# NVlabs/FoundationPose

Measured on AMD Instinct MI355X. Metric: pose-hypotheses/sec (raster+refine+score), 252 hyp x 160x160 @ 640x480 RGB-D, higher is better.
Workload: dtype f16

## Files before the change

### foundationpose_amd/csrc/conv_sw.hip

```cpp
#include <hip/hip_fp16.h>
#include <stdlib.h>
#include <string.h>
#include <type_traits>
#include "igemm_common.h"
#include "igemm_epilogue.h"

#ifdef FP_PROFILE_BUILD
__device__ unsigned long long sw_dbg[8];
extern "C" int fp_dbg_conv_sw(unsigned long long* out, int reset) {
  if (reset) { unsigned long long z[8] = {0, 0, 0, 0, 0, 0, ~0ull, 0}; return (int)hipMemcpyToSymbol(HIP_SYMBOL(sw_dbg), z, sizeof(z)); }
  return (int)hipMemcpyFromSymbol(out, HIP_SYMBOL(sw_dbg), 8 * sizeof(unsigned long long));
}
extern "C" int fp_dbg_conv_sw_epilogue(unsigned long long* out, int reset) {
  if (reset) { unsigned long long z[8] = {0, 0, 0, 0, 0, 0, 0, 0}; return (int)hipMemcpyToSymbol(HIP_SYMBOL(ig_epi_dbg), z, sizeof(z)); }
  return (int)hipMemcpyFromSymbol(out, HIP_SYMBOL(ig_epi_dbg), 8 * sizeof(unsigned long long));
}
#define SW_CLK(t) const unsigned long long t = wall_clock64()
#else
#define SW_CLK(t)
#endif

#ifndef SW_DEFAULT_VARIANT
#define SW_DEFAULT_VARIANT 0
#endif

namespace {

constexpr int SW_BK = 32, SW_NSTW = 4;
constexpr int sw_prows(int BM) { return BM == 256 ? 512 : 768; }

template <int N>
__device__ __forceinline__ void sw_wait_vm() {
  static_assert(N >= 0 && N < 64, "vmcnt is a 6-bit field");
  asm volatile("s_waitcnt vmcnt(%0)" ::"n"(N) : "memory");
}

typedef float sw_float4 __attribute__((ext_vector_type(4)));
__device__ __forceinline__ void sw_mfma16(sw_float4& acc, const half8& a, const half8& b) {
  asm volatile("v_mfma_f32_16x16x32_f16 %0, %1, %2, %0" : "+v"(acc) : "v"(a), "v"(b));
}

__device__ __forceinline__ int sw_q(const IgemmGeom& g, int m) {
  const int b = ig_fastdiv(m, g.mulP, g.shrP);
  const int r = m - b * g.HoWo;
  const int oy = ig_fastdiv(r, g.mulW, g.shrW);
  const int ox = r - oy * g.Wo;
  return (b * g.Hp + oy) * g.Wp + ox;
}

template <int BM, int BN, int TM, bool S16>
__global__ __launch_bounds__(512, 1) void k_conv_sw(IgemmParams p) {
  constexpr int BK = SW_BK, NW = 8, THREADS = 512;
  constexpr int NWN = BN / 64;
  static_assert((BM / (32 * TM)) * NWN == NW, "8 waves");
  constexpr int ROWB = BK * 2;
  constexpr int W_BYTES = BN * ROWB;
  constexpr int SW_PROWS = sw_prows(BM);
  constexpr int SW_PATCH_BYTES = SW_PROWS * ROWB;
  constexpr int WI = BN / 16 / NW;
  constexpr int PI = SW_PROWS / 16 / NW;
  static_assert(WI >= 1 && PI >= 1 && PI <= 7 && SW_PROWS == PI * 16 * NW, "tile shape");
  constexpr int STAGES_BYTES = 2 * SW_PATCH_BYTES + SW_NSTW * W_BYTES;
  constexpr int LDS_MAIN = ig_lds_main_slim<BM, BN>(STAGES_BYTES);
  auto swz = [](int row) { return (row >> 2) & 3; };
  auto swzp = [](int row) { return S16 ? (row >> 1) & 2 : (row >> 2) & 3; };
  extern __shared__ __attribute__((aligned(16))) unsigned char smem[];
  SW_CLK(t_start);
  unsigned char* const patch = smem;
  unsigned char* const wring = smem + 2 * SW_PATCH_BYTES;
  const int tid = threadIdx.x, lane = tid & 63;
  const int wid = __builtin_amdgcn_readfirstlane(tid >> 6);
  const int grp = wid >> 2;
  const int wm = wid / NWN, wn = wid - wm * NWN;
  float* bias_lds = reinterpret_cast<float*>(smem + LDS_MAIN);

  const int tiles_n = p.N / BN;
  const int nwg = gridDim.x;
  const int xcd = blockIdx.x & 7, loc = blockIdx.x >> 3;
  const int qd8 = nwg >> 3, r8 = nwg & 7;
  const int tile = (xcd < r8 ? xcd * (qd8 + 1) : r8 * (qd8 + 1) + (xcd - r8) * qd8) + loc;
  const int bm = tile / tiles_n, bn = tile - bm * tiles_n;
  const int m0 = bm * BM, n0 = bn * BN;
  const int Cin = p.Cin, Ktot = 9 * Cin, Wp = p.in.Wp;
  const int ncc = Cin / BK;
  ig_bias_to_lds(p, n0, bias_lds, wid, lane);

  const int q0 = sw_q(p.in, m0);
  const int qmax = (p.M / p.in.HoWo) * p.in.Hp * Wp - 1;
  unsigned poff32[PI], woff32[WI];
#pragma unroll
  for (int j = 0; j < PI; ++j) {
    const int row = (wid * PI + j) * 16 + (lane >> 2);
    const int c = (lane & 3) ^ swzp(row);
    int q = q0 + row;
    q = q < qmax ? q : qmax;
    poff32[j] = (unsigned)(((long long)q * p.in.cstride + p.in.coff + c * 8) * 2);
  }
#pragma unroll
  for (int j = 0; j < WI; ++j) {
    const int row = (wid * WI + j) * 16 + (lane >> 2);
    const int c = (lane & 3) ^ swz(row);
    woff32[j] = (unsigned)((((size_t)(n0 + row) * Ktot) + c * 8) * 2);
  }
  const bool wpk = (BN == 128) && p.Wpk != nullptr;
  if (wpk) {
#pragma unroll
    for (int j = 0; j < WI; ++j) woff32[j] = (unsigned)(((wid * WI + j) * 64 + lane) * 16);
  }
  const int wpk_base = wpk ? bn * (ncc * 9) * W_BYTES : 0;
  const __amdgpu_buffer_rsrc_t rsA = __builtin_amdgcn_make_buffer_rsrc(const_cast<_Float16*>(p.A), 0, 0x7FFFFFFF, 0x00020000);
  const __amdgpu_buffer_rsrc_t rsW = __builtin_amdgcn_make_buffer_rsrc(const_cast<_Float16*>(wpk ? p.Wpk : p.Wt), 0, 0x7FFFFFFF, 0x00020000);

  auto stage_patch = [&](int cc, int j) {
    unsigned char* dst = patch + (cc & 1) * SW_PATCH_BYTES + (wid * PI + j) * 1024;
    __builtin_amdgcn_raw_ptr_buffer_load_lds(rsA, (__attribute__((address_space(3))) void*)dst, 16, (int)poff32[j],
                                             cc * (BK * 2), 0, 0);
  };
  auto stage_w = [&](int cc, int tap, int slot) {
    const int wsoff = wpk ? wpk_base + (cc * 9 + tap) * W_BYTES : (tap * Cin + cc * BK) * 2;
    unsigned char* dst = wring + slot * W_BYTES + wid * (WI * 1024);
#pragma unroll
    for (int j = 0; j < WI; ++j)
      __builtin_amdgcn_raw_ptr_buffer_load_lds(rsW, (__attribute__((address_space(3))) void*)(dst + j * 1024), 16,
                                               (int)woff32[j], wsoff, 0, 0);
  };

  constexpr int NFA = S16 ? 2 * TM : TM, NFW = S16 ? 4 : 2;
  constexpr int FR = S16 ? 16 : 32;
  typedef float float4_ __attribute__((ext_vector_type(4)));
  typedef typename std::conditional<S16, float4_, float16_>::type acc_t;
  acc_t acc[NFW][NFA];
#pragma unroll
  for (int i = 0; i < NFW; ++i)
#pragma unroll
    for (int j = 0; j < NFA; ++j)
#pragma unroll
      for (int e = 0; e < (S16 ? 4 : 16); ++e) acc[i][j][e] = 0.f;

  const int frow = lane & (FR - 1), fhalf = lane >> (S16 ? 4 : 5);
  int arow[NFA], w_off[2][2];
#pragma unroll
  for (int t = 0; t < NFA; ++t) {
    int m = m0 + wm * (32 * TM) + t * FR + frow;
    m = m < p.M ? m : p.M - 1;
    arow[t] = sw_q(p.in, m) - q0;
    if constexpr (S16) arow[t] = (arow[t] << 6) + (fhalf << 4);
  }
  if constexpr (S16) {
    const int quad = (0x1320 >> (4 * (frow >> 2))) & 3;
#pragma unroll
    for (int t = 0; t < 4; ++t) {
      const int rw = wn * 64 + t * 16 + 4 * quad + (frow & 3);
      w_off[t >> 1][t & 1] = rw * ROWB + ((fhalf ^ swz(rw)) << 4);
    }
  } else {
#pragma unroll
    for (int t = 0; t < 2; ++t) {
      const int rw = wn * 64 + t * 32 + frow;
#pragma unroll
      for (int kk = 0; kk < 2; ++kk) w_off[t][kk] = rw * ROWB + (((2 * kk + fhalf) ^ swz(rw)) << 4);
    }
  }

#pragma unroll
  for (int j = 0; j < PI; ++j) stage_patch(0, j);
  stage_w(0, 0, 0);
  stage_w(0, 1, 1);
  stage_w(0, 2, 2);
  sw_wait_vm<2 * WI>();
  __builtin_amdgcn_s_barrier();
  SW_CLK(t_cold);
  if (grp) __builtin_amdgcn_s_barrier();

  half8 fa[2][TM], fw[2][2];
  static_assert(TM == 4, "the fragment addresses of the next tap are computed behind the MFMA groups of a k-step, one per group of four");
  int anext[NFA], aflip[NFA];
#pragma unroll
  for (int t = 0; t < NFA; ++t) {
    anext[t] = S16 ? arow[t] : (arow[t] << 6) + ((fhalf ^ swz(arow[t])) << 4);
    aflip[t] = S16 ? (arow[t] >> 3) & 32 : 0;
  }
  auto kstep = [&](int cc, auto tap_c, auto last_c) {
    constexpr int T = decltype(tap_c)::value;
    constexpr bool LAST = decltype(last_c)::value;
    constexpr int ky = T / 3, kx = T - 3 * ky;
    const int s = cc * 9 + T;
    const unsigned char* pb = patch + (cc & 1) * SW_PATCH_BYTES;
    const unsigned char* wb = wring + (s & (SW_NSTW - 1)) * W_BYTES;
    const int shift = ky * Wp + kx;
    if constexpr (S16) {
#pragma unroll
      for (int t = 0; t < NFA; ++t) fa[t >> 2][t & 3] = *reinterpret_cast<const half8*>(pb + (anext[t] ^ aflip[t]));
#pragma unroll
      for (int t = 0; t < 4; ++t) fw[t >> 1][t & 1] = *reinterpret_cast<const half8*>(wb + w_off[t >> 1][t & 1]);
    } else {
#pragma unroll
      for (int t = 0; t < TM; ++t) {
        const int a0 = anext[t];
        fa[0][t] = *reinterpret_cast<const half8*>(pb + a0);
        fa[1][t] = *reinterpret_cast<const half8*>(pb + (a0 ^ 32));
      }
#pragma unroll
      for (int kk = 0; kk < 2; ++kk)
#pragma unroll
        for (int t = 0; t < 2; ++t) fw[kk][t] = *reinterpret_cast<const half8*>(wb + w_off[t][kk]);
    }
    (void)shift;
    if constexpr (!LAST) {
      if constexpr (T < PI) stage_patch(cc + 1, T);
      if constexpr (T + 3 < 9) stage_w(cc, T + 3, (s + 3) & (SW_NSTW - 1));
      else stage_w(cc + 1, T - 6, (s + 3) & (SW_NSTW - 1));
      constexpr int NP = (T < PI ? 1 : 0) + ((T >= 1 && T - 1 < PI) ? 1 : 0);
      sw_wait_vm<2 * WI + NP>();
    } else {
      if constexpr (T + 3 < 9) stage_w(cc, T + 3, (s + 3) & (SW_NSTW - 1));
      constexpr int NYOUNGER = T <= 5 ? 2 : (T == 6 ? 1 : 0);
      sw_wait_vm<NYOUNGER * WI>();
    }
    asm volatile("s_waitcnt lgkmcnt(0)" ::: "memory");
    __builtin_amdgcn_sched_barrier(0);
    __builtin_amdgcn_s_barrier();
    __builtin_amdgcn_sched_barrier(0);
    __builtin_amdgcn_s_setprio(1);
    {
      constexpr int TN = (T + 1) % 9, kyn = TN / 3, kxn = TN - 3 * kyn;
      const int shift_n = kyn * Wp + kxn;
      if constexpr (S16) {
        int sh = shift_n << 6;
        asm volatile("" : "+s"(sh));
#pragma unroll
        for (int i = 0; i < 4; ++i)
#pragma unroll
          for (int jh = 0; jh < 2; ++jh) {
            const int t = i * 2 + jh;
            int x, y;
            sw_mfma16(acc[i][jh * 4 + 0], fw[i >> 1][i & 1], fa[jh][0]);
            asm volatile("v_add_u32 %0, %1, %2" : "=v"(x) : "s"(sh), "v"(arow[t]));
            sw_mfma16(acc[i][jh * 4 + 1], fw[i >> 1][i & 1], fa[jh][1]);
            asm volatile("v_lshrrev_b32 %0, 3, %1" : "=v"(y) : "v"(x));
            sw_mfma16(acc[i][jh * 4 + 2], fw[i >> 1][i & 1], fa[jh][2]);
            asm volatile("v_and_b32 %0, 32, %0" : "+v"(y));
            sw_mfma16(acc[i][jh * 4 + 3], fw[i >> 1][i & 1], fa[jh][3]);
            anext[t] = x; aflip[t] = y;
          }
      } else {
#pragma unroll
      for (int kk = 0; kk < 2; ++kk)
#pragma unroll
        for (int i = 0; i < 2; ++i) {
#pragma unroll
          for (int j = 0; j < TM; ++j)
            acc[i][j] = __builtin_amdgcn_mfma_f32_32x32x16_f16(fw[kk][i], fa[kk][j], acc[i][j], 0, 0, 0);
          const int t = kk * 2 + i;
          {
            int ar = arow[t];
            asm volatile("" : "+v"(ar));
            const int pr = ar + shift_n;
            anext[t] = (pr << 6) + ((fhalf ^ swz(pr)) << 4);
          }
        }
      }
    }
    __builtin_amdgcn_s_setprio(0);
    __builtin_amdgcn_sched_barrier(0);
    __builtin_amdgcn_s_barrier();
    __builtin_amdgcn_sched_barrier(0);
  };
  auto chunk = [&](int cc, auto last_c) {
    kstep(cc, std::integral_constant<int, 0>{}, last_c);
    kstep(cc, std::integral_constant<int, 1>{}, last_c);
    kstep(cc, std::integral_constant<int, 2>{}, last_c);
    kstep(cc, std::integral_constant<int, 3>{}, last_c);
    kstep(cc, std::integral_constant<int, 4>{}, last_c);
    kstep(cc, std::integral_constant<int, 5>{}, last_c);
    kstep(cc, std::integral_constant<int, 6>{}, last_c);
    kstep(cc, std::integral_constant<int, 7>{}, last_c);
    kstep(cc, std::integral_constant<int, 8>{}, last_c);
  };
  for (int cc = 0; cc + 1 < ncc; ++cc) chunk(cc, std::false_type{});
  chunk(ncc - 1, std::true_type{});
  if (!grp) __builtin_amdgcn_s_barrier();
  __syncthreads();
  SW_CLK(t_loop);
  ig_epilogue<BM, BN, TM, THREADS, 0, true>(p, acc, smem, m0, n0, wm, wn, tid, lane, bias_lds);
#ifdef FP_PROFILE_BUILD
  asm volatile("s_waitcnt vmcnt(0)" ::: "memory");
  SW_CLK(t_end);
  if (tid == 0) {
    atomicAdd(&sw_dbg[0], t_cold - t_start); atomicAdd(&sw_dbg[1], t_loop - t_cold); atomicAdd(&sw_dbg[2], t_end - t_loop);
    atomicAdd(&sw_dbg[3], 1ull); atomicMin(&sw_dbg[6], t_start); atomicMax(&sw_dbg[7], t_end);
  }
#endif
}

constexpr int LS_PROWS = 448, LS_NSTW = 3;

template <int BM, int BN, int TM>
__global__ __launch_bounds__(256, 2) void k_conv_sw_ls(IgemmParams p) {
  constexpr int BK = SW_BK, NW = 4, THREADS = 256;
  constexpr int NWN = BN / 64;
  static_assert((BM / (32 * TM)) * NWN == NW, "4 waves");
  constexpr int ROWB = BK * 2;
  constexpr int W_BYTES = BN * ROWB;
  constexpr int PATCH_BYTES = LS_PROWS * ROWB;
  constexpr int WI = BN / 16 / NW;
  constexpr int PI = LS_PROWS / 16 / NW;
  static_assert(WI >= 1 && PI >= 1 && PI <= 8 && LS_PROWS == PI * 16 * NW, "tile shape");
  constexpr int STAGES_BYTES = 2 * PATCH_BYTES + LS_NSTW * W_BYTES;
  static_assert(STAGES_BYTES >= BM * BN * 2 + BM * 16 + IG_BIAS_LDS, "the epilogue tile, its tables and the vectors reuse the staging area");
  auto swz = [](int row) { return (row >> 2) & 3; };
  extern __shared__ __attribute__((aligned(16))) unsigned char smem[];
  unsigned char* const patch = smem;
  unsigned char* const wring = smem + 2 * PATCH_BYTES;
  const int tid = threadIdx.x, lane = tid & 63;
  const int wid = __builtin_amdgcn_readfirstlane(tid >> 6);
  const int wm = wid / NWN, wn = wid - wm * NWN;

  const int tiles_n = p.N / BN;
  const int nwg = gridDim.x;
  const int xcd = blockIdx.x & 7, loc = blockIdx.x >> 3;
  const int qd8 = nwg >> 3, r8 = nwg & 7;
  const int tile = (xcd < r8 ? xcd * (qd8 + 1) : r8 * (qd8 + 1) + (xcd - r8) * qd8) + loc;
  const int bm = tile / tiles_n, bn = tile - bm * tiles_n;
  const int m0 = bm * BM, n0 = bn * BN;
  const int Cin = p.Cin, Ktot = 9 * Cin, Wp = p.in.Wp;
  const int ncc = Cin / BK;

  const int q0 = sw_q(p.in, m0);
  const int qmax = (p.M / p.in.HoWo) * p.in.Hp * Wp - 1;
  unsigned poff32[PI], woff32[WI];
#pragma unroll
  for (int j = 0; j < PI; ++j) {
    const int row = (wid * PI + j) * 16 + (lane >> 2);
    const int c = (lane & 3) ^ swz(row);
    int q = q0 + row;
    q = q < qmax ? q : qmax;
    poff32[j] = (unsigned)(((long long)q * p.in.cstride + p.in.coff + c * 8) * 2);
  }
#pragma unroll
  for (int j = 0; j < WI; ++j) {
    const int row = (wid * WI + j) * 16 + (lane >> 2);
    const int c = (lane & 3) ^ swz(row);
    woff32[j] = (unsigned)((((size_t)(n0 + row) * Ktot) + c * 8) * 2);
  }
  const __amdgpu_buffer_rsrc_t rsA = __builtin_amdgcn_make_buffer_rsrc(const_cast<_Float16*>(p.A), 0, 0x7FFFFFFF, 0x00020000);
  const __amdgpu_buffer_rsrc_t rsW = __builtin_amdgcn_make_buffer_rsrc(const_cast<_Float16*>(p.Wt), 0, 0x7FFFFFFF, 0x00020000);

  auto stage_patch = [&](int cc, int j) {
    unsigned char* dst = patch + (cc & 1) * PATCH_BYTES + (wid * PI + j) * 1024;
    __builtin_amdgcn_raw_ptr_buffer_load_lds(rsA, (__attribute__((address_space(3))) void*)dst, 16, (int)poff32[j],
                                             cc * (BK * 2), 0, 0);
  };
  auto stage_w = [&](int cc, int tap, int slot) {
    const int wsoff = (tap * Cin + cc * BK) * 2;
    unsigned char* dst = wring + slot * W_BYTES + wid * (WI * 1024);
#pragma unroll
    for (int j = 0; j < WI; ++j)
      __builtin_amdgcn_raw_ptr_buffer_load_lds(rsW, (__attribute__((address_space(3))) void*)(dst + j * 1024), 16,
                                               (int)woff32[j], wsoff, 0, 0);
  };

  float16_ acc[2][TM];
#pragma unroll
  for (int i = 0; i < 2; ++i)
#pragma unroll
    for (int j = 0; j < TM; ++j)
#pragma unroll
      for (int e = 0; e < 16; ++e) acc[i][j][e] = 0.f;

  const int frow = lane & 31, fhalf = lane >> 5;
  int arow[TM], w_off[2][2];
#pragma unroll
  for (int t = 0; t < TM; ++t) {
// ... 67 lines not shown
    kstep(cc, std::integral_constant<int, 0>{}, last_c, first_c);
    kstep(cc, std::integral_constant<int, 1>{}, last_c, std::false_type{});
    kstep(cc, std::integral_constant<int, 2>{}, last_c, std::false_type{});
    kstep(cc, std::integral_constant<int, 3>{}, last_c, std::false_type{});
    kstep(cc, std::integral_constant<int, 4>{}, last_c, std::false_type{});
    kstep(cc, std::integral_constant<int, 5>{}, last_c, std::false_type{});
    kstep(cc, std::integral_constant<int, 6>{}, last_c, std::false_type{});
    kstep(cc, std::integral_constant<int, 7>{}, last_c, std::false_type{});
    kstep(cc, std::integral_constant<int, 8>{}, last_c, std::false_type{});
  };
  chunk(0, std::false_type{}, std::true_type{});
  for (int cc = 1; cc + 1 < ncc; ++cc) chunk(cc, std::false_type{}, std::false_type{});
  chunk(ncc - 1, std::true_type{}, std::false_type{});
  __syncthreads();
  float* bias_lds = reinterpret_cast<float*>(smem + BM * BN * 2 + BM * 16);
  ig_bias_to_lds(p, n0, bias_lds, wid, lane);
  asm volatile("s_waitcnt vmcnt(0)" ::: "memory");
  ig_epilogue<BM, BN, TM, THREADS, 0>(p, acc, smem, m0, n0, wm, wn, tid, lane, bias_lds);
}

template <int BM, int BN, int TM>
int sw_ls_launch(const IgemmParams& p, hipStream_t stream) {
  constexpr int LDS = 2 * LS_PROWS * SW_BK * 2 + LS_NSTW * BN * SW_BK * 2;
  static_assert(2 * LDS <= 160 * 1024, "two workgroups per CU");
  const long long tiles = (long long)fp_cdiv(p.M, BM) * (p.N / BN);
  FP_REQUIRE(tiles < (1ll << 31), "fp_igemm_f16_fwd: too many tiles");
  FP_SET_MAX_LDS((k_conv_sw_ls<BM, BN, TM>), LDS);
  hipLaunchKernelGGL((k_conv_sw_ls<BM, BN, TM>), dim3((unsigned)tiles), dim3(256), LDS, stream, p);
  FP_CHECK_LAUNCH("fp_igemm_f16_fwd(conv_sw_ls)");
  return FP_OK;
}

constexpr int sw_lds_bytes(int BM, int BN) {
  return (BM == 256 ? ig_lds_main_slim<256, 256>(2 * sw_prows(256) * SW_BK * 2 + SW_NSTW * 256 * SW_BK * 2)
                    : ig_lds_main_slim<512, 128>(2 * sw_prows(512) * SW_BK * 2 + SW_NSTW * 128 * SW_BK * 2)) + IG_BIAS_LDS;
}

template <int BM, int BN, int TM, bool S16>
int sw_launch(const IgemmParams& p, hipStream_t stream) {
  static_assert((BM == 256 && BN == 256) || (BM == 512 && BN == 128), "tile shapes of sw_lds_bytes");
  constexpr int LDS = sw_lds_bytes(BM, BN);
  static_assert(LDS <= 160 * 1024, "does not fit the 160 KiB LDS");
  const long long tiles = (long long)fp_cdiv(p.M, BM) * (p.N / BN);
  FP_REQUIRE(tiles < (1ll << 31), "fp_igemm_f16_fwd: too many tiles");
  FP_SET_MAX_LDS((k_conv_sw<BM, BN, TM, S16>), LDS);
  hipLaunchKernelGGL((k_conv_sw<BM, BN, TM, S16>), dim3((unsigned)tiles), dim3(512), LDS, stream, p);
  FP_CHECK_LAUNCH("fp_igemm_f16_fwd(conv_sw)");
  return FP_OK;
}

}

static int sw_span(const IgemmGeom& g, int BM) {
  const int row_cross = (BM - 1) / g.Wo + 1, img_cross = (BM - 1) / g.HoWo + 1;
  return (BM - 1) + 2 * row_cross + (2 * g.Wp + 2) * img_cross + 2 * g.Wp + 3;
}

static int sw_variant(const IgemmParams& p) {
  int v = SW_DEFAULT_VARIANT;
#ifdef FP_PROFILE_BUILD
  static int forced = -2;
  if (forced == -2) {
    const char* e = getenv("FP_CONV_SW");
    forced = e ? (!strcmp(e, "ls") ? 1 : (!strcmp(e, "pp") ? 0 : -1)) : -1;
  }
  if (forced >= 0) v = forced;
#endif
  if (v == 2) v = p.Cin <= 128 ? 1 : 0;
  if (v == 3) v = p.Cin <= 256 ? 1 : 0;
  if (v == 1 && sw_span(p.in, 256) > LS_PROWS) v = 0;
  return v;
}

#ifndef SW_FORCE_512
#define SW_FORCE_512 1
#endif
static bool sw_use_256(const IgemmParams& p) { return (p.N % 256) == 0 && (!SW_FORCE_512 || p.M < 2 * 512); }
static int sw_tile_rows(const IgemmParams& p) { return sw_variant(p) == 1 ? 256 : (sw_use_256(p) ? 256 : 512); }

bool fp_conv3x3_sw_applicable(const IgemmParams& p) {
  const IgemmGeom& g = p.in;
  if (p.taps != 9 || g.stride != 1 || g.off != 0 || g.bsplit != 0) return false;
  if (g.HoWo % g.Wo != 0 || g.Wp != g.Wo + 2 || g.Hp != g.HoWo / g.Wo + 2) return false;
  const int BM = sw_tile_rows(p);
  if (p.M % g.HoWo != 0 || p.M < 2 * BM) return false;
  if (p.Cin % 64 != 0 || p.N % 128 != 0) return false;
  const long long bytes = (long long)(p.M / g.HoWo) * g.Hp * g.Wp * g.cstride * 2;
  if (bytes >= (1ll << 31)) return false;
  const IgemmGeom& o = p.out;
  const long long imgs = o.bsplit > 0 ? o.bsplit : p.M / g.HoWo, groups = o.bsplit > 0 ? (p.M / g.HoWo) / o.bsplit + 1 : 0;
  if (imgs * o.Hp * o.Wp * o.cstride + o.coff + groups * (long long)o.cgroup >= (1ll << 31)) return false;
  if (p.R) {
    const IgemmGeom& r = p.res;
    const long long rimgs = r.bsplit > 0 ? r.bsplit : p.M / g.HoWo, rgroups = r.bsplit > 0 ? (p.M / g.HoWo) / r.bsplit + 1 : 0;
    if (rimgs * r.Hp * r.Wp * r.cstride + r.coff + rgroups * (long long)r.cgroup >= (1ll << 31)) return false;
  }
  return sw_span(g, BM) <= (sw_variant(p) == 1 ? LS_PROWS : sw_prows(BM));
}

int fp_conv3x3_sw_tile_rows(const IgemmParams& p) { return sw_tile_rows(p); }

extern "C" int fp_conv3x3_sw_lds_bytes(void) { return sw_lds_bytes(512, 128); }

int fp_conv3x3_sw_launch(const IgemmParams& p, hipStream_t stream) {
  if (sw_variant(p) == 1) return sw_ls_launch<256, 128, 4>(p, stream);
  if (sw_use_256(p)) return p.mfma16 ? sw_launch<256, 256, 4, true>(p, stream) : sw_launch<256, 256, 4, false>(p, stream);
  return p.mfma16 ? sw_launch<512, 128, 4, true>(p, stream) : sw_launch<512, 128, 4, false>(p, stream);
}

__global__ __launch_bounds__(256) void k_pack_conv3x3_tiles(const _Float16* __restrict__ w, _Float16* __restrict__ out, int N, int Cin) {
  const int nk = 9 * (Cin / 32);
  const long long total = (long long)N * nk * 4;
  const long long q = (long long)blockIdx.x * 256 + threadIdx.x;
  if (q >= total) return;
  const int pc = (int)(q & 3);
  const int r = (int)((q >> 2) & 127);
  const long long blk = q >> 9;
  const int s = (int)(blk % nk), bn = (int)(blk / nk);
  const int cc = s / 9, tap = s - 9 * cc;
  const int lc = pc ^ ((r >> 2) & 3);
  const half8 v = *reinterpret_cast<const half8*>(w + (size_t)(bn * 128 + r) * (9 * Cin) + tap * Cin + cc * 32 + lc * 8);
  *reinterpret_cast<half8*>(out + q * 8) = v;
}

extern "C" int fp_pack_conv3x3_tiles_f16(const void* w, void* w_tiles, int N, int Cin, void* stream) {
  FP_REQUIRE(w && w_tiles && w != w_tiles, "fp_pack_conv3x3_tiles_f16: NULL tensor or in-place repack");
  FP_REQUIRE(N > 0 && N % 128 == 0 && Cin > 0 && Cin % 32 == 0, "fp_pack_conv3x3_tiles_f16: N=%d must be a multiple of 128, Cin=%d of 32", N, Cin);
  FP_REQUIRE((((size_t)w | (size_t)w_tiles) & 15) == 0, "fp_pack_conv3x3_tiles_f16: tensors must be 16-byte aligned");
  const long long total = (long long)N * 9 * (Cin / 32) * 4;
  hipLaunchKernelGGL(k_pack_conv3x3_tiles, dim3((unsigned)((total + 255) / 256)), dim3(256), 0, (hipStream_t)stream, (const _Float16*)w,
                     (_Float16*)w_tiles, N, Cin);
  FP_CHECK_LAUNCH("fp_pack_conv3x3_tiles_f16");
  return FP_OK;
}
```

### foundationpose_amd/csrc/igemm_common.h

```cpp
#pragma once
#include <hip/hip_fp16.h>
#include "fp_common.h"

typedef _Float16 half8 __attribute__((ext_vector_type(8)));
typedef _Float16 half4 __attribute__((ext_vector_type(4)));
typedef float float16_ __attribute__((ext_vector_type(16)));

#define IG_BK 64
#ifndef SW_DEFAULT_MFMA16
#define SW_DEFAULT_MFMA16 1
#endif

struct IgemmGeom {
  int HoWo, Wo;
  int Hp, Wp;
  int stride;
  int off;
  int cstride;
  int coff;
  int bsplit;
  int cgroup;
  unsigned mulP, shrP;
  unsigned mulW, shrW;
  unsigned mulB, shrB;
};

static inline void ig_fastdiv_init(int d, unsigned* mul, unsigned* shr) {
  if (d <= 1) { *mul = 0; *shr = 0; return; }
  int lg = 0;
  while ((1u << lg) < (unsigned)d) ++lg;
  const int p = 31 + lg;
  *mul = (unsigned)(((1ull << p) + (unsigned)d - 1) / (unsigned)d);
  *shr = (unsigned)(p - 32);
}
__device__ __forceinline__ int ig_fastdiv(int n, unsigned mul, unsigned shr) {
  return mul ? (int)(__umulhi((unsigned)n, mul) >> shr) : n;
}

struct IgemmParams {
  const _Float16* A;
  const _Float16* Wt;
  const _Float16* Wpk;
  const float* bias;
  const float* bn_scale;
  const float* bn_shift;
  const _Float16* R;
  _Float16* Y;
  const float* pe;
  _Float16* Ype;
  int pe_period;
  int M, N, Cin, taps;
  int relu;
  int round_acc;
  IgemmGeom in, out, res;
  int mfma16;
  int epi;
  unsigned pe_mul, pe_shr;
  float* slab;
  int nsplit;
};

#define IG_EPI_SPEC 1
#define IG_EPI_ROUND_ACC 2
#define IG_EPI_BIAS 4
#define IG_EPI_BN 8
#define IG_EPI_RES 16
#define IG_EPI_RELU 32
#define IG_EPI_PE 64
#define IG_EPI_CONV (IG_EPI_SPEC | IG_EPI_ROUND_ACC | IG_EPI_BIAS | IG_EPI_RELU)

__device__ __forceinline__ long long ig_row_off(const IgemmGeom& g, int m) {
  const int b = ig_fastdiv(m, g.mulP, g.shrP);
  const int r = m - b * g.HoWo;
  const int oy = ig_fastdiv(r, g.mulW, g.shrW);
  const int ox = r - oy * g.Wo;
  int bb = b, cg = 0;
  if (g.bsplit > 0) { cg = ig_fastdiv(b, g.mulB, g.shrB); bb = b - cg * g.bsplit; }
  return (((long long)bb * g.Hp + (oy * g.stride + g.off)) * g.Wp + (ox * g.stride + g.off)) * g.cstride + g.coff +
         (long long)cg * g.cgroup;
}
```

### foundationpose_amd/csrc/igemm_epilogue.h

```cpp
#pragma once
#include <type_traits>
#include "igemm_common.h"

#ifdef FP_PROFILE_BUILD
static __device__ unsigned long long ig_epi_dbg[8];
#define IG_CLK(t) const unsigned long long t = wall_clock64()
#else
#define IG_CLK(t)
#endif

#define IG_VEC_FLOATS 256
#define IG_BIAS_LDS (3 * IG_VEC_FLOATS * 4)

template <int BM, int BN>
constexpr int ig_lds_main(int stage_bytes) {
  return stage_bytes > BM * BN * 2 + BM * 16 ? stage_bytes : BM * BN * 2 + BM * 16;
}

template <int BM, int BN>
constexpr int ig_lds_main_slim(int stage_bytes) {
  return stage_bytes > BM * BN * 2 + BM * 4 ? stage_bytes : BM * BN * 2 + BM * 4;
}
#define IG_ROW_NONE ((int)0x80000000)

typedef float ig_float4 __attribute__((ext_vector_type(4)));
struct IgEpiArgs {
  IgemmGeom out, res;
  const _Float16* R;
  _Float16* Y;
  const float* pe;
  _Float16* Ype;
  int pe_period;
  unsigned pe_mul, pe_shr;
  int N;
};

template <typename T>
__device__ __forceinline__ T* ig_uniform_ptr(const T* ptr) {
  const unsigned long long a = reinterpret_cast<unsigned long long>(ptr);
  const unsigned lo = __builtin_amdgcn_readfirstlane((unsigned)a), hi = __builtin_amdgcn_readfirstlane((unsigned)(a >> 32));
  return reinterpret_cast<T*>(((unsigned long long)hi << 32) | lo);
}

__device__ __forceinline__ half8 ig_relu8(const half8& v) {
  typedef _Float16 half2_ __attribute__((ext_vector_type(2)));
  half8 r;
#pragma unroll
  for (int e = 0; e < 4; ++e) {
    const half2_ x = {v[2 * e], v[2 * e + 1]};
    half2_ y;
    asm("v_pk_max_f16 %0, %1, 0" : "=v"(y) : "v"(x));
    r[2 * e] = y[0]; r[2 * e + 1] = y[1];
  }
  return r;
}

template <int BM, int BN, int TM, int THREADS, bool SLIM, int EPI, typename Acc>
__device__ __forceinline__ void ig_epilogue_spec(const IgEpiArgs& p, Acc& acc, unsigned char* smem, int m0, int n0,
                                                 int wm, int wn, int tid, int lane, const float* bias_lds) {
  constexpr bool S16 = std::is_same<Acc, ig_float4[4][2 * TM]>::value;
  static_assert(S16 || std::is_same<Acc, float16_[2][TM]>::value, "accumulator layout");
  static_assert((EPI & IG_EPI_SPEC) && (EPI & IG_EPI_BIAS), "a layer kind with a bias");
  constexpr bool ROUND_ACC = (EPI & IG_EPI_ROUND_ACC) != 0, HAS_BN = (EPI & IG_EPI_BN) != 0, RES = (EPI & IG_EPI_RES) != 0;
  constexpr bool RELU = (EPI & IG_EPI_RELU) != 0, PE = (EPI & IG_EPI_PE) != 0;
  static_assert(ROUND_ACC || !HAS_BN, "BatchNorm follows the conv rounding");
  constexpr int CPR = BN / 8;
  constexpr int NIT = (BM * CPR) / THREADS;
  constexpr int RPI = THREADS / CPR;
  static_assert(THREADS % CPR == 0 && RPI % 16 == 0 && NIT * RPI == BM, "the store loop's swizzle term must not depend on the iteration");
  constexpr int ROWB = 2 * BN;
  typedef float float4_ __attribute__((ext_vector_type(4)));
  typedef _Float16 half2_ __attribute__((ext_vector_type(2)));
  typedef unsigned uint4_ __attribute__((ext_vector_type(4)));
  unsigned char* E = smem;
  long long* rowY = reinterpret_cast<long long*>(smem + BM * ROWB);
  long long* rowR = SLIM ? reinterpret_cast<long long*>(smem) : rowY + BM;
  int* rowY32 = reinterpret_cast<int*>(smem + BM * ROWB);
  const long long baseY = SLIM ? ig_row_off(p.out, m0) + n0 : 0;
  IG_CLK(te0);
  for (int r = tid; r < BM; r += THREADS) {
    const int m = m0 + r;
    if constexpr (SLIM) rowY32[r] = (int)(ig_row_off(p.out, m) + n0 - baseY);
    else rowY[r] = ig_row_off(p.out, m) + n0;
    if constexpr (RES) rowR[r] = ig_row_off(p.res, m) + n0;
  }
  __syncthreads();
  IG_CLK(te1);
  const int ml0 = tid / CPR, ch = tid % CPR;
  half8 rv[RES ? NIT : 1];
  if constexpr (RES) {
    if constexpr (SLIM) {
      const __amdgpu_buffer_rsrc_t rsR = __builtin_amdgcn_make_buffer_rsrc(ig_uniform_ptr(p.R), 0, -1, 0x00020000);
      const int* rR = reinterpret_cast<const int*>(rowR + ml0);
#pragma unroll
      for (int it = 0; it < NIT; ++it)
        rv[it] = __builtin_bit_cast(half8, __builtin_amdgcn_raw_buffer_load_b128(rsR, (int)(((unsigned)rR[it * RPI * 2] + ch * 8) << 1), 0, 0));
      __builtin_amdgcn_sched_barrier(0);
      asm volatile("s_waitcnt lgkmcnt(0)" ::: "memory");
      __builtin_amdgcn_s_barrier();
      __builtin_amdgcn_sched_barrier(0);
    } else {
      const long long* rR = rowR + ml0;
#pragma unroll
      for (int it = 0; it < NIT; ++it) rv[it] = *reinterpret_cast<const half8*>(p.R + rR[it * RPI] + ch * 8);
    }
  }
  IG_CLK(te2);
  struct Vecs { float4_ bv, sc, sh; half2_ b01, b23; };
  auto vecs = [&](int nl) {
    Vecs c;
    c.bv = *reinterpret_cast<const float4_*>(bias_lds + nl);
    c.b01 = half2_{(_Float16)c.bv[0], (_Float16)c.bv[1]};
    c.b23 = half2_{(_Float16)c.bv[2], (_Float16)c.bv[3]};
    if constexpr (HAS_BN) {
      c.sc = *reinterpret_cast<const float4_*>(bias_lds + IG_VEC_FLOATS + nl);
      c.sh = *reinterpret_cast<const float4_*>(bias_lds + 2 * IG_VEC_FLOATS + nl);
    }
    return c;
  };
  auto put4 = [&](unsigned char* dst, float a0, float a1, float a2, float a3, const Vecs& c) {
    half4 v;
    if constexpr (ROUND_ACC) {
      half2_ t01 = {(_Float16)a0, (_Float16)a1};
      half2_ t23 = {(_Float16)a2, (_Float16)a3};
      t01 = t01 + c.b01;
      t23 = t23 + c.b23;
      if constexpr (HAS_BN) {
        v[0] = (_Float16)fmaf((float)t01[0], c.sc[0], c.sh[0]);
        v[1] = (_Float16)fmaf((float)t01[1], c.sc[1], c.sh[1]);
        v[2] = (_Float16)fmaf((float)t23[0], c.sc[2], c.sh[2]);
        v[3] = (_Float16)fmaf((float)t23[1], c.sc[3], c.sh[3]);
      } else {
        v[0] = t01[0]; v[1] = t01[1]; v[2] = t23[0]; v[3] = t23[1];
      }
    } else {
      v[0] = (_Float16)(a0 + c.bv[0]); v[1] = (_Float16)(a1 + c.bv[1]); v[2] = (_Float16)(a2 + c.bv[2]); v[3] = (_Float16)(a3 + c.bv[3]);
    }
    *reinterpret_cast<half4*>(dst) = v;
  };
  const int r15 = lane & 15;
  if constexpr (S16) {
    const int quad = (0x1320 >> (4 * (lane >> 4))) & 3;
    unsigned char* Erow = E + (wm * (32 * TM) + r15) * ROWB + ((quad & 1) << 3);
    const int cx = (wn * 8 + (quad >> 1)) ^ r15;
#pragma unroll
    for (int i = 0; i < 4; ++i) {
      const Vecs c = vecs(wn * 64 + i * 16 + 4 * quad);
      unsigned char* Ei = Erow + ((cx ^ (2 * i)) << 4);
#pragma unroll
      for (int j = 0; j < 2 * TM; ++j) put4(Ei + j * (16 * ROWB), acc[i][j][0], acc[i][j][1], acc[i][j][2], acc[i][j][3], c);
    }
  } else {
    unsigned char* Erow = E + (wm * (32 * TM) + (lane & 31)) * ROWB + ((lane >> 5) << 3);
    const int cx = (wn * 8) ^ r15;
#pragma unroll
    for (int i = 0; i < 2; ++i) {
#pragma unroll
      for (int g = 0; g < 4; ++g) {
        const Vecs c = vecs(wn * 64 + i * 32 + 8 * g + 4 * (lane >> 5));
        unsigned char* Ei = Erow + ((cx ^ (4 * i + g)) << 4);
#pragma unroll
        for (int j = 0; j < TM; ++j)
          put4(Ei + j * (32 * ROWB), acc[i][j][g * 4 + 0], acc[i][j][g * 4 + 1], acc[i][j][g * 4 + 2], acc[i][j][g * 4 + 3], c);
      }
    }
  }
  __syncthreads();
  IG_CLK(te3);
  const unsigned char* Erd = E + ml0 * ROWB + ((ch ^ (ml0 & 15)) << 4);
  const __amdgpu_buffer_rsrc_t rsY = __builtin_amdgcn_make_buffer_rsrc(ig_uniform_ptr(p.Y), 0, -1, 0x00020000);
  const unsigned cbY = ((unsigned)baseY + ch * 8) << 1;
#pragma unroll
  for (int it = 0; it < NIT; ++it) {
    half8 v = *reinterpret_cast<const half8*>(Erd + it * (RPI * ROWB));
    if constexpr (RES) v = v + rv[it];
    if constexpr (RELU) v = ig_relu8(v);
    if constexpr (SLIM) __builtin_amdgcn_raw_buffer_store_b128(__builtin_bit_cast(uint4_, v), rsY, (int)(cbY + ((unsigned)rowY32[ml0 + it * RPI] << 1)), 0, 0);
    else *reinterpret_cast<half8*>(p.Y + rowY[ml0 + it * RPI] + ch * 8) = v;
    if constexpr (PE) {
      const int m = m0 + ml0 + it * RPI;
      const int mp = m - ig_fastdiv(m, p.pe_mul, p.pe_shr) * p.pe_period;
      const float* per = p.pe + (size_t)mp * p.N + n0 + ch * 8;
      const float4_ e0 = *reinterpret_cast<const float4_*>(per), e1 = *reinterpret_cast<const float4_*>(per + 4);
      half8 w;
#pragma unroll
      for (int e = 0; e < 4; ++e) { w[e] = (_Float16)((float)v[e] + e0[e]); w[4 + e] = (_Float16)((float)v[4 + e] + e1[e]); }
      *reinterpret_cast<half8*>(p.Ype + (size_t)m * p.N + n0 + ch * 8) = w;
      __builtin_amdgcn_sched_barrier(0);
    }
  }
#ifdef FP_PROFILE_BUILD
  IG_CLK(te4);
  if (tid == 0) {
    atomicAdd(&ig_epi_dbg[0], te1 - te0); atomicAdd(&ig_epi_dbg[1], te2 - te1); atomicAdd(&ig_epi_dbg[2], te3 - te2);
    atomicAdd(&ig_epi_dbg[3], te4 - te3); atomicAdd(&ig_epi_dbg[4], 1ull);
  }
#endif
}
template <int BM, int BN, int TM, int THREADS, int DBG, bool FULL, bool SLIM, int EPI = 0, typename Acc, typename P>
__device__ __forceinline__ void ig_epilogue_body(const P& p, Acc& acc, unsigned char* smem, int m0, int n0,
                                                 int wm, int wn, int tid, int lane, const float* bias_lds) {
  if constexpr (EPI != 0) {
    static_assert(FULL && std::is_same<P, IgEpiArgs>::value, "the layer-kind bodies take whole tiles and their own argument block");
    ig_epilogue_spec<BM, BN, TM, THREADS, SLIM, EPI>(p, acc, smem, m0, n0, wm, wn, tid, lane, bias_lds);
  } else {
  static_assert(std::is_same<P, IgemmParams>::value, "the generic body reads IgemmParams");
  constexpr bool S16 = std::is_same<Acc, ig_float4[4][2 * TM]>::value;
  static_assert(S16 || std::is_same<Acc, float16_[2][TM]>::value, "accumulator layout");
  constexpr int CPR = BN / 8;
  constexpr int NIT = (BM * CPR) / THREADS;
  unsigned char* E = smem;
  typedef float float4_ __attribute__((ext_vector_type(4)));
  const bool round_acc = p.round_acc != 0, has_bn = p.bn_scale != nullptr;
  long long* rowY = reinterpret_cast<long long*>(smem + BM * 2 * BN);
  long long* rowR = SLIM ? reinterpret_cast<long long*>(smem) : rowY + BM;
  int* rowY32 = reinterpret_cast<int*>(smem + BM * 2 * BN);
  const long long baseY = SLIM ? ig_row_off(p.out, m0) + n0 : 0;
  auto row_exists = [&](int ml) { return SLIM ? rowY32[ml] != IG_ROW_NONE : rowY[ml] >= 0; };
  IG_CLK(te0);
  for (int r = tid; r < BM; r += THREADS) {
    const int m = m0 + r;
    const bool in = m < p.M;
    if constexpr (SLIM) rowY32[r] = in ? (int)(ig_row_off(p.out, m) + n0 - baseY) : IG_ROW_NONE;
    else rowY[r] = in ? ig_row_off(p.out, m) + n0 : -1;
    if (p.R) rowR[r] = in ? ig_row_off(p.res, m) + n0 : 0;
  }
  __syncthreads();
  IG_CLK(te1);
  half8 rv[NIT];
  if (p.R) {
#pragma unroll
    for (int it = 0; it < NIT; ++it) {
      const int qd = tid + it * THREADS;
      const int ml = qd / CPR, ch = qd % CPR;
      if (FULL || row_exists(ml)) rv[it] = *reinterpret_cast<const half8*>(p.R + rowR[ml] + ch * 8);
    }
    if constexpr (SLIM) {
      __builtin_amdgcn_sched_barrier(0);
      asm volatile("s_waitcnt lgkmcnt(0)" ::: "memory");
      __builtin_amdgcn_s_barrier();
      __builtin_amdgcn_sched_barrier(0);
// ... 35 lines not shown
    const int quad = (0x1320 >> (4 * (lane >> 4))) & 3;
#pragma unroll
    for (int i = 0; i < 4; ++i) {
      const int nl = wn * 64 + i * 16 + 4 * quad;
      float4_ bv, sc, sh;
      vecs(nl, bv, sc, sh);
#pragma unroll
      for (int j = 0; j < 2 * TM; ++j) {
        const int ml = wm * (32 * TM) + j * 16 + (lane & 15);
        put4(nl, ml, acc[i][j][0], acc[i][j][1], acc[i][j][2], acc[i][j][3], bv, sc, sh);
      }
    }
  } else {
#pragma unroll
    for (int i = 0; i < 2; ++i) {
#pragma unroll
      for (int g = 0; g < 4; ++g) {
        const int nl = wn * 64 + i * 32 + 8 * g + 4 * (lane >> 5);
        float4_ bv, sc, sh;
        vecs(nl, bv, sc, sh);
#pragma unroll
        for (int j = 0; j < TM; ++j) {
          const int ml = wm * (32 * TM) + j * 32 + (lane & 31);
          put4(nl, ml, acc[i][j][g * 4 + 0], acc[i][j][g * 4 + 1], acc[i][j][g * 4 + 2], acc[i][j][g * 4 + 3], bv, sc, sh);
        }
      }
    }
  }
  __syncthreads();
  IG_CLK(te3);
  const half8 zero = {0, 0, 0, 0, 0, 0, 0, 0};
#pragma unroll
  for (int it = 0; it < NIT; ++it) {
    const int qd = tid + it * THREADS;
    const int ml = qd / CPR, ch = qd % CPR;
    if (!FULL && !row_exists(ml)) continue;
    const long long yo = SLIM ? baseY + rowY32[ml] : rowY[ml];
    half8 v = *reinterpret_cast<const half8*>(E + ml * (2 * BN) + ((ch ^ (ml & 15)) << 4));
    if (p.R) v = v + rv[it];
    if (p.relu) v = __builtin_elementwise_max(v, zero);
    *reinterpret_cast<half8*>(p.Y + yo + ch * 8) = v;
    if (p.Ype) {
      const int m = m0 + ml;
      const float* per = p.pe + (size_t)(m % p.pe_period) * p.N + n0 + ch * 8;
      const float4_ e0 = *reinterpret_cast<const float4_*>(per), e1 = *reinterpret_cast<const float4_*>(per + 4);
      half8 w;
#pragma unroll
      for (int e = 0; e < 4; ++e) { w[e] = (_Float16)((float)v[e] + e0[e]); w[4 + e] = (_Float16)((float)v[4 + e] + e1[e]); }
      *reinterpret_cast<half8*>(p.Ype + (size_t)m * p.N + n0 + ch * 8) = w;
    }
  }
#ifdef FP_PROFILE_BUILD
  IG_CLK(te4);
  if (tid == 0) {
    atomicAdd(&ig_epi_dbg[0], te1 - te0); atomicAdd(&ig_epi_dbg[1], te2 - te1); atomicAdd(&ig_epi_dbg[2], te3 - te2);
    atomicAdd(&ig_epi_dbg[3], te4 - te3); atomicAdd(&ig_epi_dbg[4], 1ull);
  }
#endif
  }
}

template <int BM, int BN, int TM, int THREADS, int DBG = 0, bool SLIM = false, typename Acc>
__device__ __forceinline__ void ig_epilogue(const IgemmParams& p, Acc& acc, unsigned char* smem, int m0, int n0,
                                            int wm, int wn, int tid, int lane, const float* bias_lds) {
  if (m0 + BM <= p.M) {
    if constexpr (DBG == 0) {
#define IG_EPI_CASE(E) case E: ig_epilogue_body<BM, BN, TM, THREADS, DBG, true, SLIM, E>(q, acc, smem, m0, n0, wm, wn, tid, lane, bias_lds); return
      const IgEpiArgs q = {p.out, p.res, p.R, p.Y, p.pe, p.Ype, p.pe_period, p.pe_mul, p.pe_shr, p.N};
      switch (p.epi) {
        IG_EPI_CASE(IG_EPI_CONV);
        IG_EPI_CASE(IG_EPI_CONV | IG_EPI_RES);
        IG_EPI_CASE(IG_EPI_CONV | IG_EPI_RES | IG_EPI_PE);
        IG_EPI_CASE(IG_EPI_CONV | IG_EPI_BN);
        IG_EPI_CASE(IG_EPI_CONV | IG_EPI_BN | IG_EPI_RES);
        IG_EPI_CASE(IG_EPI_CONV | IG_EPI_BN | IG_EPI_RES | IG_EPI_PE);
        default: break;
      }
#undef IG_EPI_CASE
    }
    ig_epilogue_body<BM, BN, TM, THREADS, DBG, true, SLIM>(p, acc, smem, m0, n0, wm, wn, tid, lane, bias_lds);
  }
  else ig_epilogue_body<BM, BN, TM, THREADS, DBG, false, SLIM>(p, acc, smem, m0, n0, wm, wn, tid, lane, bias_lds);
}
__device__ __forceinline__ void ig_bias_to_lds(const IgemmParams& p, int n0, float* bias_lds, int wid, int lane) {
  if (wid > 2) return;
  const float* src = wid == 0 ? p.bias : (wid == 1 ? p.bn_scale : p.bn_shift);
  float* dst = bias_lds + wid * IG_VEC_FLOATS;
  if (src) {
    const __amdgpu_buffer_rsrc_t rs = __builtin_amdgcn_make_buffer_rsrc(const_cast<float*>(src), 0, p.N * 4, 0x00020000);
    __builtin_amdgcn_raw_ptr_buffer_load_lds(rs, (__attribute__((address_space(3))) void*)dst, 16, lane * 16, n0 * 4, 0, 0);
  } else if (wid == 0) {
    typedef float f4 __attribute__((ext_vector_type(4)));
    *reinterpret_cast<f4*>(dst + lane * 4) = f4{0.f, 0.f, 0.f, 0.f};
  }
}
```

Before: 7864.

## Shorten conv_sw prologue: hoist params, issue first loads early, interleave residual loads

The sliding-window conv kernel now reads its fields from a reordered IgemmParams head into scalar registers up front. It computes the grid size from M/N instead of gridDim, and uses a shift for the tile split when tiles_n is a power of two. Patch and weight loads for the first stage are issued before the fragment-address setup, which is pinned with asm barriers so address math overlaps load latency. The epilogue spreads residual buffer loads across the accumulator-to-LDS write groups instead of issuing them all at once. New guards on Wo and cstride keep the unsigned 32-bit offset arithmetic valid.

```diff
diff --git a/foundationpose_amd/csrc/conv_sw.hip b/foundationpose_amd/csrc/conv_sw.hip
--- a/foundationpose_amd/csrc/conv_sw.hip
+++ b/foundationpose_amd/csrc/conv_sw.hip
@@ -40,10 +40,18 @@
   asm volatile("v_mfma_f32_16x16x32_f16 %0, %1, %2, %0" : "+v"(acc) : "v"(a), "v"(b));
 }
 
-__device__ __forceinline__ int sw_q(const IgemmGeom& g, int m) {
-  const int b = ig_fastdiv(m, g.mulP, g.shrP);
+__device__ __forceinline__ int sw_div(int n, unsigned mul, unsigned shr) { return (int)(__umulhi((unsigned)n, mul) >> shr); }
+
+struct SwGeom {
+  int HoWo, Wo, Hp, Wp;
+  unsigned mulP, shrP, mulW, shrW;
+};
+
+template <typename G>
+__device__ __forceinline__ int sw_q(const G& g, int m) {
+  const int b = sw_div(m, g.mulP, g.shrP);
   const int r = m - b * g.HoWo;
-  const int oy = ig_fastdiv(r, g.mulW, g.shrW);
+  const int oy = sw_div(r, g.mulW, g.shrW);
   const int ox = r - oy * g.Wo;
   return (b * g.Hp + oy) * g.Wp + ox;
 }
@@ -74,27 +82,43 @@
   const int wm = wid / NWN, wn = wid - wm * NWN;
   float* bias_lds = reinterpret_cast<float*>(smem + LDS_MAIN);
 
-  const int tiles_n = p.N / BN;
-  const int nwg = gridDim.x;
+  const _Float16* A_ = p.A;
+  const _Float16* W_ = p.Wt;
+  const _Float16* Wpk_ = p.Wpk;
+  const float* bias_ = p.bias;
+  const float* bnsc_ = p.bn_scale;
+  const float* bnsh_ = p.bn_shift;
+  const int M = p.M, N = p.N, Cin = p.Cin, cstride = p.in.cstride, coff = p.in.coff;
+  const SwGeom gi = {p.in.HoWo, p.in.Wo, p.in.Hp, p.in.Wp, p.in.mulP, p.in.shrP, p.in.mulW, p.in.shrW};
+  asm volatile("" ::"s"(A_), "s"(W_), "s"(Wpk_), "s"(bias_), "s"(bnsc_), "s"(bnsh_), "s"(M), "s"(N), "s"(Cin), "s"(cstride), "s"(coff),
+               "s"(gi.HoWo), "s"(gi.Wo), "s"(gi.Hp), "s"(gi.Wp), "s"(gi.mulP), "s"(gi.shrP), "s"(gi.mulW), "s"(gi.shrW));
+  __builtin_amdgcn_sched_barrier(0);
+
+  const int tiles_n = N / BN;
+  const int nwg = (int)(((unsigned)M + BM - 1) / BM) * tiles_n;
   const int xcd = blockIdx.x & 7, loc = blockIdx.x >> 3;
   const int qd8 = nwg >> 3, r8 = nwg & 7;
   const int tile = (xcd < r8 ? xcd * (qd8 + 1) : r8 * (qd8 + 1) + (xcd - r8) * qd8) + loc;
-  const int bm = tile / tiles_n, bn = tile - bm * tiles_n;
+  const int bm = __builtin_popcount(tiles_n) == 1 ? tile >> __builtin_ctz(tiles_n) : tile / tiles_n, bn = tile - bm * tiles_n;
   const int m0 = bm * BM, n0 = bn * BN;
-  const int Cin = p.Cin, Ktot = 9 * Cin, Wp = p.in.Wp;
+  const int Ktot = 9 * Cin, Wp = gi.Wp;
   const int ncc = Cin / BK;
-  ig_bias_to_lds(p, n0, bias_lds, wid, lane);
-
-  const int q0 = sw_q(p.in, m0);
-  const int qmax = (p.M / p.in.HoWo) * p.in.Hp * Wp - 1;
+  ig_bias_to_lds(bias_, bnsc_, bnsh_, N, n0, bias_lds, wid, lane);
+
+  const int q0 = sw_q(gi, m0);
+  const int qmax = sw_div(M, gi.mulP, gi.shrP) * gi.Hp * Wp - 1;
   unsigned poff32[PI], woff32[WI];
-#pragma unroll
-  for (int j = 0; j < PI; ++j) {
-    const int row = (wid * PI + j) * 16 + (lane >> 2);
-    const int c = (lane & 3) ^ swzp(row);
-    int q = q0 + row;
-    q = q < qmax ? q : qmax;
-    poff32[j] = (unsigned)(((long long)q * p.in.cstride + p.in.coff + c * 8) * 2);
+  {
+    const int row0 = wid * PI * 16 + (lane >> 2);
+    const int c = (lane & 3) ^ swzp(row0);
+    static_assert(((16 >> 1) & 2) == 0 && ((16 >> 2) & 3) == 0, "swzp(row0 + 16 j) == swzp(row0)");
+    const unsigned ps2 = (unsigned)cstride * 2, omax = (unsigned)qmax * ps2, lane_off = (unsigned)(coff + c * 8) * 2;
+    const unsigned o0 = (unsigned)(q0 + row0) * ps2;
+#pragma unroll
+    for (int j = 0; j < PI; ++j) {
+      const unsigned o = o0 + j * 16 * ps2;
+      poff32[j] = (o < omax ? o : omax) + lane_off;
+    }
   }
 #pragma unroll
   for (int j = 0; j < WI; ++j) {
@@ -102,14 +126,14 @@
     const int c = (lane & 3) ^ swz(row);
     woff32[j] = (unsigned)((((size_t)(n0 + row) * Ktot) + c * 8) * 2);
   }
-  const bool wpk = (BN == 128) && p.Wpk != nullptr;
+  const bool wpk = (BN == 128) && Wpk_ != nullptr;
   if (wpk) {
 #pragma unroll
     for (int j = 0; j < WI; ++j) woff32[j] = (unsigned)(((wid * WI + j) * 64 + lane) * 16);
   }
   const int wpk_base = wpk ? bn * (ncc * 9) * W_BYTES : 0;
-  const __amdgpu_buffer_rsrc_t rsA = __builtin_amdgcn_make_buffer_rsrc(const_cast<_Float16*>(p.A), 0, 0x7FFFFFFF, 0x00020000);
-  const __amdgpu_buffer_rsrc_t rsW = __builtin_amdgcn_make_buffer_rsrc(const_cast<_Float16*>(wpk ? p.Wpk : p.Wt), 0, 0x7FFFFFFF, 0x00020000);
+  const __amdgpu_buffer_rsrc_t rsA = __builtin_amdgcn_make_buffer_rsrc(const_cast<_Float16*>(A_), 0, 0x7FFFFFFF, 0x00020000);
+  const __amdgpu_buffer_rsrc_t rsW = __builtin_amdgcn_make_buffer_rsrc(const_cast<_Float16*>(wpk ? Wpk_ : W_), 0, 0x7FFFFFFF, 0x00020000);
 
   auto stage_patch = [&](int cc, int j) {
     unsigned char* dst = patch + (cc & 1) * SW_PATCH_BYTES + (wid * PI + j) * 1024;
@@ -124,6 +148,14 @@
       __builtin_amdgcn_raw_ptr_buffer_load_lds(rsW, (__attribute__((address_space(3))) void*)(dst + j * 1024), 16,
                                                (int)woff32[j], wsoff, 0, 0);
   };
+
+#pragma unroll
+  for (int j = 0; j < PI; ++j) stage_patch(0, j);
+  stage_w(0, 0, 0);
+  stage_w(0, 1, 1);
+  stage_w(0, 2, 2);
+  __builtin_amdgcn_sched_barrier(0);
+  SW_CLK(t_issue);
 
   constexpr int NFA = S16 ? 2 * TM : TM, NFW = S16 ? 4 : 2;
   constexpr int FR = S16 ? 16 : 32;
@@ -142,8 +174,8 @@
 #pragma unroll
   for (int t = 0; t < NFA; ++t) {
     int m = m0 + wm * (32 * TM) + t * FR + frow;
-    m = m < p.M ? m : p.M - 1;
-    arow[t] = sw_q(p.in, m) - q0;
+    m = m < M ? m : M - 1;
+    arow[t] = sw_q(gi, m) - q0;
     if constexpr (S16) arow[t] = (arow[t] << 6) + (fhalf << 4);
   }
   if constexpr (S16) {
@@ -161,25 +193,32 @@
       for (int kk = 0; kk < 2; ++kk) w_off[t][kk] = rw * ROWB + (((2 * kk + fhalf) ^ swz(rw)) << 4);
     }
   }
-
-#pragma unroll
-  for (int j = 0; j < PI; ++j) stage_patch(0, j);
-  stage_w(0, 0, 0);
-  stage_w(0, 1, 1);
-  stage_w(0, 2, 2);
+  static_assert(TM == 4, "the fragment addresses of the next tap are computed behind the MFMA groups of a k-step, one per group of four");
+  int anext[NFA], aflip[NFA];
+#pragma unroll
+  for (int t = 0; t < NFA; ++t) {
+    anext[t] = S16 ? arow[t] : (arow[t] << 6) + ((fhalf ^ swz(arow[t])) << 4);
+    aflip[t] = S16 ? (arow[t] >> 3) & 32 : 0;
+  }
+
+#pragma unroll
+  for (int t = 0; t < NFA; ++t) {
+    asm volatile("" : "+v"(arow[t]), "+v"(anext[t]));
+    if constexpr (S16) asm volatile("" : "+v"(aflip[t]));
+  }
+  asm volatile("" : "+v"(w_off[0][0]), "+v"(w_off[0][1]), "+v"(w_off[1][0]), "+v"(w_off[1][1]));
+#pragma unroll
+  for (int i = 0; i < NFW; ++i)
+#pragma unroll
+    for (int j = 0; j < NFA; ++j) asm volatile("" : "+v"(acc[i][j]));
+  __builtin_amdgcn_sched_barrier(0);
+
   sw_wait_vm<2 * WI>();
   __builtin_amdgcn_s_barrier();
   SW_CLK(t_cold);
   if (grp) __builtin_amdgcn_s_barrier();
 
   half8 fa[2][TM], fw[2][2];
-  static_assert(TM == 4, "the fragment addresses of the next tap are computed behind the MFMA groups of a k-step, one per group of four");
-  int anext[NFA], aflip[NFA];
-#pragma unroll
-  for (int t = 0; t < NFA; ++t) {
-    anext[t] = S16 ? arow[t] : (arow[t] << 6) + ((fhalf ^ swz(arow[t])) << 4);
-    aflip[t] = S16 ? (arow[t] >> 3) & 32 : 0;
-  }
   auto kstep = [&](int cc, auto tap_c, auto last_c) {
     constexpr int T = decltype(tap_c)::value;
     constexpr bool LAST = decltype(last_c)::value;
@@ -288,7 +327,7 @@
   SW_CLK(t_end);
   if (tid == 0) {
     atomicAdd(&sw_dbg[0], t_cold - t_start); atomicAdd(&sw_dbg[1], t_loop - t_cold); atomicAdd(&sw_dbg[2], t_end - t_loop);
-    atomicAdd(&sw_dbg[3], 1ull); atomicMin(&sw_dbg[6], t_start); atomicMax(&sw_dbg[7], t_end);
+    atomicAdd(&sw_dbg[3], 1ull); atomicAdd(&sw_dbg[4], t_issue - t_start); atomicMin(&sw_dbg[6], t_start); atomicMax(&sw_dbg[7], t_end);
   }
 #endif
 }
@@ -522,11 +561,13 @@
   const IgemmGeom& g = p.in;
   if (p.taps != 9 || g.stride != 1 || g.off != 0 || g.bsplit != 0) return false;
   if (g.HoWo % g.Wo != 0 || g.Wp != g.Wo + 2 || g.Hp != g.HoWo / g.Wo + 2) return false;
+  if (g.Wo < 2) return false;
   const int BM = sw_tile_rows(p);
   if (p.M % g.HoWo != 0 || p.M < 2 * BM) return false;
   if (p.Cin % 64 != 0 || p.N % 128 != 0) return false;
   const long long bytes = (long long)(p.M / g.HoWo) * g.Hp * g.Wp * g.cstride * 2;
   if (bytes >= (1ll << 31)) return false;
+  if (g.cstride >= (1 << 19)) return false;
   const IgemmGeom& o = p.out;
   const long long imgs = o.bsplit > 0 ? o.bsplit : p.M / g.HoWo, groups = o.bsplit > 0 ? (p.M / g.HoWo) / o.bsplit + 1 : 0;
   if (imgs * o.Hp * o.Wp * o.cstride + o.coff + groups * (long long)o.cgroup >= (1ll << 31)) return false;
diff --git a/foundationpose_amd/csrc/igemm_common.h b/foundationpose_amd/csrc/igemm_common.h
--- a/foundationpose_amd/csrc/igemm_common.h
+++ b/foundationpose_amd/csrc/igemm_common.h
@@ -1,5 +1,6 @@
 #pragma once
 #include <hip/hip_fp16.h>
+#include <stddef.h>
 #include "fp_common.h"
 
 typedef _Float16 half8 __attribute__((ext_vector_type(8)));
@@ -44,21 +45,23 @@
   const float* bias;
   const float* bn_scale;
   const float* bn_shift;
+  int M, N, Cin, taps;
+  IgemmGeom in;
+  IgemmGeom out, res;
   const _Float16* R;
   _Float16* Y;
   const float* pe;
   _Float16* Ype;
   int pe_period;
-  int M, N, Cin, taps;
   int relu;
   int round_acc;
-  IgemmGeom in, out, res;
   int mfma16;
   int epi;
   unsigned pe_mul, pe_shr;
   float* slab;
   int nsplit;
 };
+static_assert(sizeof(IgemmGeom) == 64 && offsetof(IgemmParams, in) == 64 && offsetof(IgemmParams, out) == 128, "the head of IgemmParams is its first 128 bytes");
 
 #define IG_EPI_SPEC 1
 #define IG_EPI_ROUND_ACC 2
diff --git a/foundationpose_amd/csrc/igemm_epilogue.h b/foundationpose_amd/csrc/igemm_epilogue.h
--- a/foundationpose_amd/csrc/igemm_epilogue.h
+++ b/foundationpose_amd/csrc/igemm_epilogue.h
@@ -88,13 +88,23 @@
   IG_CLK(te1);
   const int ml0 = tid / CPR, ch = tid % CPR;
   half8 rv[RES ? NIT : 1];
+  constexpr int NRG = S16 ? 4 : 8;
+  static_assert(NIT % NRG == 0, "residual loads per channel group");
+  unsigned roff[RES && SLIM ? NIT : 1];
+  const __amdgpu_buffer_rsrc_t rsR = __builtin_amdgcn_make_buffer_rsrc(ig_uniform_ptr(p.R), 0, -1, 0x00020000);
+  auto res_group = [&](int g) {
+    if constexpr (RES && SLIM) {
+#pragma unroll
+      for (int it = g * (NIT / NRG); it < (g + 1) * (NIT / NRG); ++it)
+        rv[it] = __builtin_bit_cast(half8, __builtin_amdgcn_raw_buffer_load_b128(rsR, (int)roff[it], 0, 0));
+      __builtin_amdgcn_sched_barrier(0);
+    }
+  };
   if constexpr (RES) {
     if constexpr (SLIM) {
-      const __amdgpu_buffer_rsrc_t rsR = __builtin_amdgcn_make_buffer_rsrc(ig_uniform_ptr(p.R), 0, -1, 0x00020000);
       const int* rR = reinterpret_cast<const int*>(rowR + ml0);
 #pragma unroll
-      for (int it = 0; it < NIT; ++it)
-        rv[it] = __builtin_bit_cast(half8, __builtin_amdgcn_raw_buffer_load_b128(rsR, (int)(((unsigned)rR[it * RPI * 2] + ch * 8) << 1), 0, 0));
+      for (int it = 0; it < NIT; ++it) roff[it] = ((unsigned)rR[it * RPI * 2] + ch * 8) << 1;
       __builtin_amdgcn_sched_barrier(0);
       asm volatile("s_waitcnt lgkmcnt(0)" ::: "memory");
       __builtin_amdgcn_s_barrier();
@@ -145,6 +155,7 @@
     const int cx = (wn * 8 + (quad >> 1)) ^ r15;
 #pragma unroll
     for (int i = 0; i < 4; ++i) {
+      res_group(i);
       const Vecs c = vecs(wn * 64 + i * 16 + 4 * quad);
       unsigned char* Ei = Erow + ((cx ^ (2 * i)) << 4);
 #pragma unroll
@@ -157,6 +168,7 @@
     for (int i = 0; i < 2; ++i) {
 #pragma unroll
       for (int g = 0; g < 4; ++g) {
+        res_group(i * 4 + g);
         const Vecs c = vecs(wn * 64 + i * 32 + 8 * g + 4 * (lane >> 5));
         unsigned char* Ei = Erow + ((cx ^ (4 * i + g)) << 4);
 #pragma unroll
@@ -358,15 +370,19 @@
   }
   else ig_epilogue_body<BM, BN, TM, THREADS, DBG, false, SLIM>(p, acc, smem, m0, n0, wm, wn, tid, lane, bias_lds);
 }
-__device__ __forceinline__ void ig_bias_to_lds(const IgemmParams& p, int n0, float* bias_lds, int wid, int lane) {
+__device__ __forceinline__ void ig_bias_to_lds(const float* bias, const float* bn_scale, const float* bn_shift, int N, int n0, float* bias_lds,
+                                               int wid, int lane) {
   if (wid > 2) return;
-  const float* src = wid == 0 ? p.bias : (wid == 1 ? p.bn_scale : p.bn_shift);
+  const float* src = wid == 0 ? bias : (wid == 1 ? bn_scale : bn_shift);
   float* dst = bias_lds + wid * IG_VEC_FLOATS;
   if (src) {
-    const __amdgpu_buffer_rsrc_t rs = __builtin_amdgcn_make_buffer_rsrc(const_cast<float*>(src), 0, p.N * 4, 0x00020000);
+    const __amdgpu_buffer_rsrc_t rs = __builtin_amdgcn_make_buffer_rsrc(const_cast<float*>(src), 0, N * 4, 0x00020000);
     __builtin_amdgcn_raw_ptr_buffer_load_lds(rs, (__attribute__((address_space(3))) void*)dst, 16, lane * 16, n0 * 4, 0, 0);
   } else if (wid == 0) {
     typedef float f4 __attribute__((ext_vector_type(4)));
     *reinterpret_cast<f4*>(dst + lane * 4) = f4{0.f, 0.f, 0.f, 0.f};
   }
 }
+__device__ __forceinline__ void ig_bias_to_lds(const IgemmParams& p, int n0, float* bias_lds, int wid, int lane) {
+  ig_bias_to_lds(p.bias, p.bn_scale, p.bn_shift, p.N, n0, bias_lds, wid, lane);
+}
```

Result: faster. 7977, median of 6 (+1.4%).
